# grahamstockton87/RayTracingOneWeekendApplication

Hardware: AMD Instinct MI355X
Metric: Msamples/sec (pixels x spp) on RTIOW final scene 1920x1080 (higher is better)
Workload: dtype f64; 1 GPU; book1_final 1920x1080x100spp depth 50 (BASELINE configs[1]); tiles=8x8 px per wave, interleaved over ranks, parallelism=1 GPU, scene_seed=1592598565, render_seed=1, program_ops=1337, reduced=False, variant=0, order=fast (rtk_scene_upload_fast; proven bit-identical), frames_in_flight=1

## Files before the change

include/rtk.h:

```cpp
#ifndef RTK_H
#define RTK_H

#include <stddef.h>
#include <stdint.h>

#ifdef __cplusplus
extern "C" {
#endif

#define RTK_ABI_VERSION 2

typedef enum rtk_status {
    RTK_OK = 0,
    RTK_ERR_INVALID = -1,
    RTK_ERR_NO_DEVICE = -2,
    RTK_ERR_HIP = -3,
    RTK_ERR_UNSUPPORTED = -4,
    RTK_ERR_NO_SCENE = -5
} rtk_status;

typedef struct rtk_vec3 { double x, y, z; } rtk_vec3;

typedef enum rtk_node_kind {
    RTK_NODE_SPHERE = 1,
// ... 487 lines not shown
int rtk_gather_irradiance_host(rtk_ctx* ctx, const rtk_gather_opts* opts, int64_t n, const double* h_points, const double* h_normals, double* h_irradiance);
int rtk_gather_occlusion_host(rtk_ctx* ctx, const rtk_gather_opts* opts, int64_t n, const double* h_points, const double* h_normals, double* h_open,
                              double* h_bent);

int rtk_debug_closest_hit(rtk_ctx* ctx, int real_mode, int n, const double* h_rays, const uint32_t* h_keys,
                          double* h_out, uint64_t* h_draws);

int rtk_debug_scatter(rtk_ctx* ctx, int real_mode, int n, const int32_t* h_materials, const double* h_rays, const double* h_records,
                      const uint32_t* h_keys, double* h_out, uint64_t* h_draws);
int rtk_debug_texture(rtk_ctx* ctx, int real_mode, int n, const int32_t* h_textures, const double* h_uvp, double* h_out, uint64_t* h_work);
int rtk_debug_get_ray(rtk_ctx* ctx, int real_mode, const rtk_camera* cam, uint32_t seed, int n, const int32_t* h_pixel_sample,
                      double* h_out, uint64_t* h_draws);

int rtk_scene_info(rtk_ctx* ctx, int32_t* n_program_ops, int64_t* bytes_f64, int64_t* bytes_f32);

int rtk_frame_launches(const rtk_camera* cam, const rtk_render_opts* opts);

const char* rtk_kernel_name(rtk_ctx* ctx, int real_mode, int variant);

int rtk_render_views(rtk_ctx* ctx, int32_t n_views, const rtk_camera* h_cams, const uint32_t* h_seeds ,
                     const rtk_render_opts* opts, void* d_linear, uint8_t* d_rgb8, rtk_work_counters* d_counters);
int rtk_render_views_host(rtk_ctx* ctx, int32_t n_views, const rtk_camera* h_cams, const uint32_t* h_seeds, const rtk_render_opts* opts,
                          double* h_linear, uint8_t* h_rgb8, rtk_work_counters* counters);
const char* rtk_view_kernel_name(rtk_ctx* ctx, int real_mode, int variant);

#ifdef __cplusplus
}
#endif
#endif
```

raytracingoneweekendapplication_amd/csrc/rtk_api.cpp:

```cpp
#include <hip/hip_runtime.h>

#include <algorithm>
#include <cmath>
#include <cstdarg>
#include <cstdio>
#include <cstdlib>
#include <cstring>
#include <map>
#include <new>
#include <string>
#include <vector>

#include "rtk.h"
#include "rtk_ctx.h"
#include "rtk_device_layout.h"
#include "rtk_internal.h"
#include "rtk_lds_plan.h"

namespace rtk {

thread_local std::string g_error;

int fail(int code, const char* fmt, ...) {
    char buf[512];
// ... 285 lines not shown
            cont[1] = 1.0 / s.radius;
            if (kind == OP_SPHERE_MOVING) {
                cont[2] = s.center_dir.x;
                cont[3] = s.center_dir.y;
                cont[4] = s.center_dir.z;
                cont[5] = s.radius * s.radius;
            } else {
                cont[2] = s.radius * s.radius;
            }
            rec->aux = (op.aux & 255u) | (uint32_t(s.material) << 8);
        }
    }
    extent_out = float(extent);
}

static double scene_extent(const rtk_scene_desc& sc, double eye_extent) {
    double e = eye_extent;
    auto take = [&](double v) { e = std::max(e, std::fabs(v)); };
    for (int32_t i = 0; i < sc.n_bvh_boxes; i++) {
        const rtk_aabb& b = sc.bvh_boxes[i];
        for (double v : {b.xmin, b.xmax, b.ymin, b.ymax, b.zmin, b.zmax}) take(v);
    }
    for (int32_t i = 0; i < sc.n_spheres; i++) {
        const rtk_sphere& s = sc.spheres[i];
        for (double c : {s.center0.x, s.center0.y, s.center0.z, s.center0.x + s.center_dir.x, s.center0.y + s.center_dir.y, s.center0.z + s.center_dir.z})
            e = std::max(e, std::fabs(c) + std::fabs(s.radius));
    }
    for (int32_t i = 0; i < sc.n_quads; i++) {
        const rtk_quad& q = sc.quads[i];
        for (int k = 0; k < 4; k++) {
// ... 359 lines not shown
    if ((rc = out.upload(slots, &out.view.program)) != RTK_OK) return rc;
    if ((rc = out.upload(tris, &out.view.tris)) != RTK_OK) return rc;
    if ((rc = out.upload(mats, &out.view.materials)) != RTK_OK) return rc;
    if ((rc = out.upload(texs, &out.view.textures)) != RTK_OK) return rc;
    if ((rc = out.upload(images, &out.view.images)) != RTK_OK) return rc;
    if ((rc = out.upload(texels, &out.view.texels)) != RTK_OK) return rc;
    if ((rc = out.upload(perlins, &out.view.perlins)) != RTK_OK) return rc;
    if ((rc = out.upload(chains, &out.view.chains)) != RTK_OK) return rc;
    if ((rc = out.upload(lights, &out.view.lights)) != RTK_OK) return rc;
    out.view.n_slots = int32_t(slots.size());
    out.view.n_lights = sc.n_lights;
    out.view.n_materials = sc.n_materials;
    out.view.n_perlins = sc.n_perlins;
    out.view.n_chains = int32_t(chains.size());
    out.view.program_mixed = nullptr;
    out.view.n_units = 0;
    out.view.extent = 0.0f;
    out.view.box_cache = nullptr;
    out.view.kind_words = nullptr;
    out.view.box_rank = nullptr;
    out.view.n_cached_boxes = out.view.n_kind_words = out.view.n_rank_words = 0;
    if (lds_plan::wants_box_table(slots.size() * sizeof(Slot<real>), mats.size() * sizeof(MaterialRec<real>))) {
        std::vector<BoxRec<real>> boxes;
        std::vector<uint32_t> kind_words((slots.size() + 7) / 8, 0u);
        std::vector<uint2> rank((slots.size() + 31) / 32, uint2{0u, 0u});
        for (size_t pc = 0; pc < slots.size();) {
            const uint32_t kind = slots[pc].kind_payload & 15u;
            kind_words[pc >> 3] |= kind << ((pc & 7) * 4);
            if (kind == OP_BOX) {
                rank[pc >> 5].x |= 1u << (pc & 31);
// ... 32 lines not shown
    if (fast_order) {
        std::vector<uint32_t> rank_of_slot(slots.size(), 0u);
        bool any = false;
        for (size_t i = 0; i < prog.ops.size(); i++) {
            rank_of_slot[slot_of_op[i]] = prog.ranks[i];
            any = any || prog.ranks[i] != 0;
        }
        if (any && (rc = out.upload(rank_of_slot, &out.view.tie_rank_slot)) != RTK_OK) return rc;
    }
    if constexpr (sizeof(real) == 8) {
        if (fast_order && want_mixed) {
            std::vector<MixedHead> units;
            std::vector<uint32_t> ranks;
            build_mixed_program(sc, prog, eye_extent, units, ranks, out.view.extent);
            if ((rc = out.upload(units, &out.view.program_mixed)) != RTK_OK) return rc;
            if ((rc = out.upload(ranks, &out.view.tie_rank)) != RTK_OK) return rc;
            out.view.n_units = int32_t(units.size());
        } else if (fast_order) {
            std::vector<Unit16> units;
            std::vector<uint32_t> ranks;
            build_compact_program(sc, prog, eye_extent, units, ranks, out.view.extent);
            if ((rc = out.upload(units, &out.view.program_compact)) != RTK_OK) return rc;
            if ((rc = out.upload(ranks, &out.view.tie_rank)) != RTK_OK) return rc;
            out.view.n_units16 = int32_t(units.size());
            out.view.compact_ch = compact_ch_family(prog) ? 1 : 0;
            if ((prog.features & ~kFeatQuadBox) != 0 && (prog.features & ~kFeatMesh) != 0) {
                std::vector<Unit16> hot, cold;
                std::vector<uint32_t> ranks_by_id;
                build_hot_cold_program(sc, prog, hot, cold, ranks_by_id);
                if (getenv("RTK_DEBUG")) fprintf(stderr, "[rtk] COMPACT program %zu B; hot part %zu B, cold part %zu B\n", units.size() * 16, hot.size() * 16, cold.size() * 16);
// ... 228 lines not shown
    RTK_HIP(hipSetDevice(ctx->device));
    ctx->has_scene = false;
    ctx->order_valid = false;
    const bool want_mixed = fast_order && prog.features == kFeatLean && prog.chains.size() <= 1;
    if ((rc = build_device_scene<double>(*scene, prog, ctx->scene64, fast_order, want_mixed, eye_extent)) != RTK_OK) return rc;
    if ((rc = build_device_scene<float>(*scene, prog, ctx->scene32, fast_order)) != RTK_OK) return rc;
    ctx->features = prog.features | hierarchy_flags;
    ctx->n_ops = int32_t(prog.ops.size());
    ctx->n_materials = scene->n_materials;
    ctx->n_textures = scene->n_textures;
    ctx->scene_digest = scene_digest(*scene, prog, ctx->features, fast_order, eye_extent);
    ctx->has_scene = true;
    return RTK_OK;
}

int rtk_scene_info(rtk_ctx* ctx, int32_t* n_program_ops, int64_t* bytes_f64, int64_t* bytes_f32) {
    if (!ctx || !ctx->has_scene) return fail(RTK_ERR_NO_SCENE, "rtk_scene_info: no scene uploaded");
    if (n_program_ops) *n_program_ops = ctx->scene64.view.n_slots;
    if (bytes_f64) *bytes_f64 = ctx->scene64.bytes;
    if (bytes_f32) *bytes_f32 = ctx->scene32.bytes;
    return RTK_OK;
}

}

namespace rtk {

size_t hot_program_lds_bytes(const rtk_scene_desc* scene) {
    if (!scene) return 0;
    try {
// ... 43 lines not shown
```

raytracingoneweekendapplication_amd/csrc/rtk_device_layout.h:

```cpp
#ifndef RTK_DEVICE_LAYOUT_H
#define RTK_DEVICE_LAYOUT_H

#include <stdint.h>
#include <hip/hip_vector_types.h>


namespace rtk {

enum OpKind : uint32_t {
    OP_END = 0,
    OP_BOX = 1,
    OP_SPHERE = 2,
    OP_QUAD = 3,
    OP_TRI = 4,
    OP_CHAIN = 5,
    OP_MED_BEGIN = 6,
    OP_MED_MID = 7,
    OP_MED_END = 8,
    OP_SPHERE_MOVING = 9,
    OP_MED_SPHERE = 10,
    OP_DEAD = 15
};

struct Op {
// ... 21 lines not shown
inline constexpr int slots_of(uint32_t kind) {
    return kind == OP_QUAD ? 3 : ((kind == OP_TRI || kind == OP_SPHERE_MOVING) ? 2 : 1);
}

struct alignas(16) MixedHead {
    uint32_t w[6];
    uint32_t kind_payload, aux;
    constexpr float f(int k) const { return __builtin_bit_cast(float, w[k]); }
    constexpr double d(int k) const { return __builtin_bit_cast(double, (unsigned long long)(w[2 * k]) | ((unsigned long long)(w[2 * k + 1]) << 32)); }
    void set_f(int k, float x) { w[k] = __builtin_bit_cast(uint32_t, x); }
    void set_d(int k, double x) {
        const unsigned long long v = __builtin_bit_cast(unsigned long long, x);
        w[2 * k] = uint32_t(v);
        w[2 * k + 1] = uint32_t(v >> 32);
    }
};
static_assert(sizeof(MixedHead) == 32, "mixed unit size");
inline constexpr int mixed_units(uint32_t kind) { return kind == OP_SPHERE ? 2 : (kind == OP_SPHERE_MOVING ? 3 : 1); }

struct alignas(16) Unit16 {
    uint32_t w[4];
};
inline constexpr int compact_units(uint32_t kind) {
    return (kind == OP_SPHERE || kind == OP_MED_SPHERE) ? 3 : (kind == OP_SPHERE_MOVING ? 5 : (kind == OP_QUAD ? 9 : (kind == OP_TRI ? 5 : 2)));
}

constexpr uint32_t kNoHit = 0xFFFFFFFFu;
constexpr int kMaxChain = 4;
constexpr int kMaxChunks = 64;
constexpr int kLdsBytesPerCU = 160 * 1024;

enum Feature : uint32_t {
// ... 74 lines not shown
template <typename real>
struct SceneView {
    const Slot<real>* program;
    const TriRec<real>* tris;
    const MaterialRec<real>* materials;
    const TextureRec<real>* textures;
    const ImageRec* images;
    const uint8_t* texels;
    const PerlinRec<real>* perlins;
    const ChainRec<real>* chains;
    const LightRec<real>* lights;
    int32_t n_slots, n_lights, n_materials;
    const MixedHead* program_mixed;
    int32_t n_units;
    float extent;
    const Unit16* program_compact;
    int32_t n_units16;
    int32_t compact_ch;
    const Unit16* program_hot;
    const Unit16* program_cold;
    int32_t n_hot_units, n_cold_units;
    const uint32_t* tie_rank_hot;
    const uint32_t* tie_rank;
    const uint32_t* tie_rank_slot;
    const BoxRec<real>* box_cache;
    const uint32_t* kind_words;
    const uint2* box_rank;
    int32_t n_cached_boxes, n_kind_words, n_rank_words;
    int32_t n_perlins, n_chains;
};
// ... 22 lines not shown
```

raytracingoneweekendapplication_amd/csrc/rtk_microbench.hip:

```cpp
#include <hip/hip_runtime.h>

#include <algorithm>
#include <cstdint>
#include <cstdio>
#include <cstring>
#include <vector>

namespace {

__global__ __launch_bounds__(256) void copy_kernel(const uint4* __restrict__ src, uint4* __restrict__ dst, size_t n) {
    for (size_t i = size_t(blockIdx.x) * 256 + threadIdx.x; i < n; i += size_t(gridDim.x) * 256) dst[i] = src[i];
}
__global__ __launch_bounds__(256) void read_kernel(const uint4* __restrict__ src, size_t n, unsigned* __restrict__ sink) {
    unsigned acc = 0;
    for (size_t i = size_t(blockIdx.x) * 256 + threadIdx.x; i < n; i += size_t(gridDim.x) * 256) {
        const uint4 v = src[i];
        acc ^= v.x ^ v.y ^ v.z ^ v.w;
    }
    if (acc == 0x12345u) *sink = acc;
}

template <bool RANDOM>
__global__ __launch_bounds__(1024) void lds_read_kernel(int iters, unsigned* __restrict__ sink) {
    extern __shared__ __align__(16) unsigned char lds[];
// ... 24 lines not shown
                                                       unsigned long long* __restrict__ real_ticks = nullptr) {
    __shared__ unsigned next[4096];
    for (int k = threadIdx.x; k < 4096; k += 64) next[k] = (k * 1031u + 17u) & 4095u;
    __syncthreads();
    unsigned at = threadIdx.x;
    const unsigned long long r0 = __builtin_amdgcn_s_memrealtime();
    const unsigned long long t0 = __builtin_amdgcn_s_memtime();
    for (int it = 0; it < iters; it++) at = next[at];
    const unsigned long long t1 = __builtin_amdgcn_s_memtime();
    const unsigned long long r1 = __builtin_amdgcn_s_memrealtime();
    if (threadIdx.x == 0) cycles[blockIdx.x] = t1 - t0;
    if (threadIdx.x == 0 && real_ticks) real_ticks[blockIdx.x] = r1 - r0;
    if (at == 0xFFFFFFFFu) *sink = at;
}

enum IssueClass { I_FMA_F32, I_FMA_F64, I_MUL_F64, I_ADD_F64, I_MUL_LO_U32, I_RCP_F32, I_SQRT_F32, I_RCP_F64, I_RSQ_F64, I_SQRT_F64, I_CNDMASK, I_MAX3_F32, I_PK_FMA_F32, I_PK_MUL_F32, I_FMAC_F32, I_MUL_F32, I_COUNT };

constexpr int kIssueReps = 16;
template <int CLS>
__global__ __launch_bounds__(1024) void issue_kernel(int iters, unsigned long long* __restrict__ cycles, float* __restrict__ sink,
                                                    unsigned long long* __restrict__ real_ticks = nullptr) {
    float f[8];
    double d[8];
    unsigned u[8];
    for (int k = 0; k < 8; k++) {
        f[k] = 1.0f + 0.001f * float(threadIdx.x + k);
        d[k] = 1.0 + 0.001 * double(threadIdx.x + k);
        u[k] = threadIdx.x * 3u + unsigned(k) + 1u;
    }
    const float fb = 0.999f, fc = 0.001f;
    const double db = 0.999, dc = 0.001;
    const unsigned um = 0x9E3779B1u;
    const unsigned long long r0 = __builtin_amdgcn_s_memrealtime();
    const unsigned long long t0 = __builtin_amdgcn_s_memtime();
    for (int it = 0; it < iters; it++) {
#pragma unroll
        for (int rep = 0; rep < kIssueReps; rep++) {
#pragma unroll
            for (int k = 0; k < 8; k++) {
                if (CLS == I_FMA_F32) asm volatile("v_fma_f32 %0, %0, %1, %2" : "+v"(f[k]) : "v"(fb), "v"(fc));
                if (CLS == I_FMA_F64) asm volatile("v_fma_f64 %0, %0, %1, %2" : "+v"(d[k]) : "v"(db), "v"(dc));
                if (CLS == I_MUL_F64) asm volatile("v_mul_f64 %0, %0, %1" : "+v"(d[k]) : "v"(db));
                if (CLS == I_ADD_F64) asm volatile("v_add_f64 %0, %0, %1" : "+v"(d[k]) : "v"(dc));
                if (CLS == I_MUL_LO_U32) asm volatile("v_mul_lo_u32 %0, %0, %1" : "+v"(u[k]) : "v"(um));
                if (CLS == I_RCP_F32) asm volatile("v_rcp_f32 %0, %0" : "+v"(f[k]));
                if (CLS == I_SQRT_F32) asm volatile("v_sqrt_f32 %0, %0" : "+v"(f[k]));
                if (CLS == I_RCP_F64) asm volatile("v_rcp_f64 %0, %0" : "+v"(d[k]));
                if (CLS == I_RSQ_F64) asm volatile("v_rsq_f64 %0, %0" : "+v"(d[k]));
                if (CLS == I_SQRT_F64) asm volatile("v_sqrt_f64 %0, %0" : "+v"(d[k]));
                if (CLS == I_CNDMASK) asm volatile("v_cndmask_b32 %0, %0, %1, vcc" : "+v"(f[k]) : "v"(fb));
                if (CLS == I_MAX3_F32) asm volatile("v_max3_f32 %0, %0, %1, %2" : "+v"(f[k]) : "v"(fb), "v"(fc));
                if (CLS == I_PK_FMA_F32) asm volatile("v_pk_fma_f32 %0, %0, %1, %2" : "+v"(d[k]) : "v"(db), "v"(dc));
                if (CLS == I_PK_MUL_F32) asm volatile("v_pk_mul_f32 %0, %0, %1" : "+v"(d[k]) : "v"(db));
                if (CLS == I_FMAC_F32) asm volatile("v_fmac_f32 %0, %1, %2" : "+v"(f[k]) : "v"(fb), "v"(fc));
                if (CLS == I_MUL_F32) asm volatile("v_mul_f32 %0, %0, %1" : "+v"(f[k]) : "v"(fb));
            }
        }
    }
    const unsigned long long t1 = __builtin_amdgcn_s_memtime();
    const unsigned long long r1 = __builtin_amdgcn_s_memrealtime();
    if (threadIdx.x == 0) cycles[blockIdx.x] = t1 - t0;
    if (threadIdx.x == 0 && real_ticks) real_ticks[blockIdx.x] = r1 - r0;
    float acc = 0.0f;
    for (int k = 0; k < 8; k++) acc += f[k] + float(d[k]) + float(u[k]);
    if (acc == 12345.678f) *sink = acc;
}

const char* kNames =
    "hbm_copy_GBps,hbm_read_GBps,lds_read_b128_GBps,lds_read_b128_random_GBps,lds_roundtrip_cycles,shader_clock_GHz,"
    "issue_v_fma_f32,issue_v_fma_f64,issue_v_mul_f64,issue_v_add_f64,issue_v_mul_lo_u32,issue_v_rcp_f32,issue_v_sqrt_f32,issue_v_rcp_f64,issue_v_rsq_f64,"
    "issue_v_sqrt_f64,issue_v_cndmask_b32,issue_v_max3_f32,issue_v_pk_fma_f32,issue_v_pk_mul_f32,issue_v_fmac_f32,issue_v_mul_f32,clock_dense_valu_GHz,clock_light_load_GHz,"
    "issue_v_fma_f32_1wave,issue_v_fma_f32_2waves,issue_v_fma_f32_4waves,issue_v_fma_f32_8waves";
constexpr int kResults = 6 + I_COUNT + 2 + 4;

#define MB_HIP(call)                                  \
    do {                                              \
        const hipError_t e_ = (call);                 \
        if (e_ != hipSuccess) {                       \
            std::snprintf(g_err, sizeof g_err, "%s: %s", #call, hipGetErrorString(e_)); \
            return -3;                                \
        }                                             \
    } while (0)
char g_err[256] = "";

template <typename F>
int time_ms(F&& launch, int reps, float* best_ms) {
// ... 116 lines not shown
    if (rc == 0) rc = run_issue<I_FMA_F64>(cus, bw, bt, d_cycles, d_real, d_fsink, &out[6 + I_FMA_F64], nullptr);
    if (rc == 0) rc = run_issue<I_MUL_F64>(cus, bw, bt, d_cycles, d_real, d_fsink, &out[6 + I_MUL_F64], nullptr);
    if (rc == 0) rc = run_issue<I_ADD_F64>(cus, bw, bt, d_cycles, d_real, d_fsink, &out[6 + I_ADD_F64], nullptr);
    if (rc == 0) rc = run_issue<I_MUL_LO_U32>(cus, bw, bt, d_cycles, d_real, d_fsink, &out[6 + I_MUL_LO_U32], nullptr);
    if (rc == 0) rc = run_issue<I_RCP_F32>(cus, bw, bt, d_cycles, d_real, d_fsink, &out[6 + I_RCP_F32], nullptr);
    if (rc == 0) rc = run_issue<I_SQRT_F32>(cus, bw, bt, d_cycles, d_real, d_fsink, &out[6 + I_SQRT_F32], nullptr);
    if (rc == 0) rc = run_issue<I_RCP_F64>(cus, bw, bt, d_cycles, d_real, d_fsink, &out[6 + I_RCP_F64], nullptr);
    if (rc == 0) rc = run_issue<I_RSQ_F64>(cus, bw, bt, d_cycles, d_real, d_fsink, &out[6 + I_RSQ_F64], nullptr);
    if (rc == 0) rc = run_issue<I_SQRT_F64>(cus, bw, bt, d_cycles, d_real, d_fsink, &out[6 + I_SQRT_F64], nullptr);
    if (rc == 0) rc = run_issue<I_CNDMASK>(cus, bw, bt, d_cycles, d_real, d_fsink, &out[6 + I_CNDMASK], nullptr);
    if (rc == 0) rc = run_issue<I_MAX3_F32>(cus, bw, bt, d_cycles, d_real, d_fsink, &out[6 + I_MAX3_F32], nullptr);
    if (rc == 0) rc = run_issue<I_PK_FMA_F32>(cus, bw, bt, d_cycles, d_real, d_fsink, &out[6 + I_PK_FMA_F32], nullptr);
    if (rc == 0) rc = run_issue<I_PK_MUL_F32>(cus, bw, bt, d_cycles, d_real, d_fsink, &out[6 + I_PK_MUL_F32], nullptr);
    if (rc == 0) rc = run_issue<I_FMAC_F32>(cus, bw, bt, d_cycles, d_real, d_fsink, &out[6 + I_FMAC_F32], nullptr);
    if (rc == 0) rc = run_issue<I_MUL_F32>(cus, bw, bt, d_cycles, d_real, d_fsink, &out[6 + I_MUL_F32], nullptr);
    if (rc == 0) {
        const int blocks = cus * bw, iters = 40000 / kIssueReps;
        for (int k = 0; k < 100; k++) issue_kernel<I_FMA_F32><<<dim3(blocks), dim3(bt), 0, nullptr>>>(iters, d_cycles, d_fsink, d_real);
        MB_HIP(hipDeviceSynchronize());
        rc = clock_from(d_cycles, d_real, blocks, &out[6 + I_COUNT]);
        if (rc == 0) {
            lds_chain_kernel<<<dim3(cus), dim3(64), 0, nullptr>>>(200000, d_cycles, sink, d_real);
            MB_HIP(hipDeviceSynchronize());
            rc = clock_from(d_cycles, d_real, cus, &out[6 + I_COUNT + 1]);
        }
    }
    (void)hipFree(d_real);
    (void)hipFree(src);
    (void)hipFree(dst);
    (void)hipFree(sink);
// ... 7 lines not shown
```

raytracingoneweekendapplication_amd/csrc/rtk_render_body.inc:

```
    extern __shared__ __align__(16) unsigned char lds_program[];
    if constexpr (IN_LDS) {
        typedef const unsigned char __attribute__((address_space(3))) * lds_bytes_t;
        if (uint32_t(size_t((lds_bytes_t)lds_program)) != 0u) return;
    }
    constexpr bool BRACKET = (FEAT_ALL & F_SPHERE_MEDIA_ONLY) == 0;
    constexpr uint32_t FEAT = FEAT_ALL & ~uint32_t(F_LDS_BOXES | F_SPHERE_MEDIA_ONLY) & ~uint32_t(RTK_DEV_MASK_OFF);
    constexpr bool LDS_PART = (FEAT_ALL & F_LDS_BOXES) != 0;
    static_assert(!LDS_PART || !IN_LDS, "F_LDS_BOXES: for programs that do not fit LDS");
    constexpr bool MIXED = (FEAT & F_F32_BOX) != 0;
    constexpr bool COMPACT = MIXED && (FEAT & ~uint32_t(F_F32_BOX | F_MATTE)) != kFeatLean;
    static_assert(!MIXED || sizeof(real) == 8, "F_F32_BOX: f64 kernels only");
    constexpr bool CH = MIXED && !COMPACT;
    constexpr bool CHE = COMPACT && kCompactChStatic<FEAT>;
    constexpr bool CHE_RT = COMPACT && COUNT && !CHE;
    [[maybe_unused]] const bool che_rt = CHE_RT && sc.compact_ch != 0;
    constexpr int kCulling = CH ? 1 : (CHE ? 2 : (CHE_RT ? 3 : 0));
    constexpr bool SPLIT = LDS_PART && !COMPACT;
    constexpr bool COLD = LDS_PART && COMPACT;
    static_assert(!LDS_PART || !MIXED || COMPACT, "F_LDS_BOXES with f32 boxes: the COMPACT program");
    constexpr bool XF = (FEAT & F_XFORM) != 0;
    using ProgRec = std::conditional_t<COMPACT, Unit16, std::conditional_t<MIXED, MixedHead, Slot<real>>>;
    using CurRec = std::conditional_t<MIXED, MixedHead, Slot<real>>;
    constexpr uint32_t kBoxUnits = COMPACT ? 2u : 1u, kSphereUnits = COMPACT ? 3u : (MIXED ? 2u : 1u), kQuadUnits = COMPACT ? 9u : 3u, kTriUnits = COMPACT ? 5u : 2u;
    const ProgRec* prog;
    if constexpr (COLD) prog = sc.program_hot;
    else if constexpr (COMPACT) prog = sc.program_compact;
    else if constexpr (MIXED) prog = sc.program_mixed;
    else prog = sc.program;
    const int n_records = COLD ? sc.n_hot_units : (COMPACT ? sc.n_units16 : (MIXED ? sc.n_units : sc.n_slots));
    [[maybe_unused]] const Unit16* cold = nullptr;
    if constexpr (COLD) cold = sc.program_cold;
    const MaterialRec<real>* mats = sc.materials;
    if constexpr (IN_LDS || COLD) {
        const int n_prog16 = n_records * int(sizeof(ProgRec) / 16);
        const int n_mat16 = sc.n_materials * int(sizeof(MaterialRec<real>) / 16);
        const uint4* __restrict__ src = reinterpret_cast<const uint4*>(prog);
        const uint4* __restrict__ msrc = reinterpret_cast<const uint4*>(sc.materials);
        uint4* dst = reinterpret_cast<uint4*>(lds_program);
        for (int k = threadIdx.x; k < n_prog16; k += blockDim.x) dst[k] = src[k];
        for (int k = threadIdx.x; k < n_mat16; k += blockDim.x) dst[n_prog16 + k] = msrc[k];
        if constexpr (COLD && (FEAT & F_TEXTURE) != 0) {
// ... 51 lines not shown
    constexpr uint32_t kPcUnit = CH ? kChPcUnit : 1u;
    auto rec_at = [&](uint32_t pc) -> const ProgRec* {
        if constexpr (CH && IN_LDS) {
            typedef const unsigned char __attribute__((address_space(3))) * lds_bytes_t;
            return reinterpret_cast<const ProgRec*>((const unsigned char*)(lds_bytes_t)(size_t)pc);
        } else if constexpr (CH) return reinterpret_cast<const ProgRec*>(reinterpret_cast<const unsigned char*>(prog) + pc);
        else return prog + pc;
    };
    auto head_at = [&](uint32_t pc) -> CurRec {
        if constexpr (COMPACT) return *reinterpret_cast<const MixedHead*>(prog + (pc & kPcMask));
        else return *rec_at(pc);
    };
    auto kind_of = [&](uint32_t pc) -> uint32_t {
        if constexpr (SPLIT) return (lds_kinds[pc >> 3] >> ((pc & 7u) * 4u)) & 15u;
        else if constexpr (COMPACT) return prog[(pc & kPcMask) + 1].w[2] & 15u;
        else return rec_at(pc)->kind_payload & 15u;
    };
    [[maybe_unused]] auto box_at = [&](uint32_t pc) -> CurRec {
        const uint2 e = lds_rank[pc >> 5];
        const uint32_t at = e.y + uint32_t(__builtin_popcount(e.x & ((1u << (pc & 31u)) - 1u)));
        if constexpr (MIXED) {
            return CurRec{};
        } else {
            const BoxRec<real> b = lds_boxes[at];
            Slot<real> s;
            #pragma unroll
            for (int k = 0; k < 6; k++) s.v[k] = b.v[k];
            s.kind_payload = OP_BOX;
            s.aux = b.aux;
            return s;
// ... 174 lines not shown
        if ((m_box | m_sph | m_oth | m_shd | m_quad | m_tri) == 0ull) {
            if (exhausted) break;
            continue;
        }
        const int n_box = popcount64(m_box), n_sph = popcount64(m_sph), n_oth = popcount64(m_oth), n_shd = popcount64(m_shd);
        const int n_quad = popcount64(m_quad), n_tri = popcount64(m_tri);
        RTK_PROF_MARK(0, 1, n_box + n_sph + n_oth + n_shd + n_quad + n_tri)
        int pick;
        if (n_box >= n_sph && n_box >= n_quad && n_box >= n_tri && n_box >= n_shd && n_box >= n_oth) pick = W_BOX;
        else if (n_sph >= n_quad && n_sph >= n_tri && n_sph >= n_shd && n_sph >= n_oth) pick = W_SPHERE;
        else if (n_quad >= n_tri && n_quad >= n_shd && n_quad >= n_oth) pick = W_QUAD;
        else if (n_tri >= n_shd && n_tri >= n_oth) pick = W_TRI;
        else if (n_shd >= n_oth) pick = W_SHADE;
        else pick = W_OTHER;
        if (pick == W_BOX) {
            const int sel = int(diag >> 8) & 7;
            const int eighths = sel == 0 ? (kFamily == kFeatMesh ? 3 : 2) : sel;
            const int frac = (n_box * eighths) >> 3;
            const int keep = frac > 8 ? frac : 8;
            constexpr int kBoxUnroll = COLD ? kUnrollCold : SPLIT ? kUnrollSplit
                                       : (((MIXED && !COMPACT) || FEAT == (kFeatLean | uint32_t(F_FMA_BOX))) ? kUnrollMixed
                                          : (kFamily == kFeatAll ? 2 : (kFamily == kFeatQuadBox ? (COMPACT ? kUnrollCompactQuadBox : kUnrollQuadBox)
                                                                       : (kFamily == kFeatMesh ? (COMPACT ? kUnrollCompactMesh : kUnrollMesh) : kUnrollLean))));
            CurRec cur;
            uint32_t k = kind;
            auto fetch = [&]() {
                if constexpr (SPLIT) {
                    k = kind_of(L.pc);
                    if (k == OP_BOX) cur = box_at(L.pc);
                } else {
// ... 69 lines not shown
                    }
                }
                if constexpr ((FEAT & ~uint32_t(F_FMA_BOX | F_F32_BOX | F_MATTE)) == kFeatQuadBox) {
                    if (popcount64(__ballot(k == OP_QUAD)) >= kQuadRide) {
                        if (k == OP_QUAD) {
                            hit_quad<XF, MIXED>(L, prog + L.pc, kQuadUnits, cnt, tie);
                            fetch();
                            L.kind = k;
                        }
                    }
                }
                remaining = popcount64(__ballot(k == box_kind));
                RTK_PROF_MARK(1, 1, remaining)
            } while (remaining >= keep);
            __builtin_amdgcn_s_setprio(0);
        } else if (pick == W_SPHERE) {
            const int ssel = int(diag >> 11) & 7;
            const int sfrac = (n_sph * (ssel == 0 ? 4 : ssel)) >> 3;
            const int keep = sfrac > 8 ? sfrac : 8;
            CurRec cur = head_at(L.pc);
            uint32_t k = kind;
            int remaining;
            __builtin_amdgcn_s_setprio(kSphereLoopPrio);
            do {
                if (k == OP_SPHERE) {
                    if constexpr (COMPACT) step_sphere_compact<XF>(L, cur, prog + L.pc, cnt, tie);
                    else if constexpr (MIXED) step_sphere_mixed<kPcUnit>(L, cur, rec_at(L.pc), cnt, tie, extent);
                    else step_sphere<XF>(L, cur, cnt, tie);
                    if constexpr (SPLIT) {
                        k = kind_of(L.pc);
                        if (k == OP_SPHERE) cur = head_at(L.pc);
                    } else {
                        cur = head_at(L.pc);
                        k = cur.kind_payload & 15u;
                    }
                    L.kind = k;
                }
                remaining = popcount64(__ballot(k == OP_SPHERE));
                RTK_PROF_MARK(2, 1, remaining)
            } while (remaining >= keep);
            __builtin_amdgcn_s_setprio(0);
        } else if ((FEAT & F_QUAD) && pick == W_QUAD) {
          if constexpr ((FEAT & F_QUAD) != 0) {
            const int keep = (n_quad >> 1) > 8 ? (n_quad >> 1) : 8;
            uint32_t k = kind;
            int remaining;
            __builtin_amdgcn_s_setprio(kPrimLoopPrio);
            do {
                if (k == OP_QUAD) {
// ... 115 lines not shown
```

raytracingoneweekendapplication_amd/csrc/rtk_trace.hip:

```cpp
#include <hip/hip_runtime.h>

#include <cstdio>
#include <cstdlib>
#include <type_traits>

#include "rtk.h"
#include "rtk_device_layout.h"
#include "rtk_device_math.h"
#include "rtk_gather_rule.h"
#include "rtk_image_pass.h"
#include "rtk_lds_plan.h"
#include "rtk_trace.h"

namespace rtk {

template <typename real> RTK_DEV V3<real> ld3(const real* p) { return V3<real>{p[0], p[1], p[2]}; }
template <typename real> RTK_DEV V3<real> operator-(V3<real> a) { return V3<real>{-a.x, -a.y, -a.z}; }
template <typename real> RTK_DEV V3<real> operator-(V3<real> a, V3<real> b) { return V3<real>{a.x - b.x, a.y - b.y, a.z - b.z}; }
template <typename real> RTK_DEV V3<real> operator*(V3<real> a, V3<real> b) { return V3<real>{a.x * b.x, a.y * b.y, a.z * b.z}; }
template <typename real> RTK_DEV V3<real> divide(V3<real> a, real t) { return scale(real(1) / t, a); }
template <typename real> RTK_DEV real dot(V3<real> a, V3<real> b) { return a.x * b.x + a.y * b.y + a.z * b.z; }
template <typename real> RTK_DEV V3<real> cross(V3<real> a, V3<real> b) {
    return V3<real>{a.y * b.z - a.z * b.y, a.z * b.x - a.x * b.z, a.x * b.y - a.y * b.x};
}
// ... 510 lines not shown
RTK_DEV float min3_clamp01(float a, float b, float c) { float r; asm("v_min3_f32 %0, %1, %2, %3 clamp" : "=v"(r) : "v"(a), "v"(b), "v"(c)); return r; }
RTK_DEV bool slab_test32_chs(const MixedHead& b, V3<float> oi, V3<float> inv) {
    const float tcx = __builtin_fmaf(b.f(0), inv.x, -oi.x), tcy = __builtin_fmaf(b.f(1), inv.y, -oi.y), tcz = __builtin_fmaf(b.f(2), inv.z, -oi.z);
    const float ax = __builtin_fabsf(inv.x), ay = __builtin_fabsf(inv.y), az = __builtin_fabsf(inv.z);
    const float nx = __builtin_fmaf(-b.f(3), ax, tcx), fx = __builtin_fmaf(b.f(3), ax, tcx);
    const float ny = __builtin_fmaf(-b.f(4), ay, tcy), fy = __builtin_fmaf(b.f(4), ay, tcy);
    const float nz = __builtin_fmaf(-b.f(5), az, tcz), fz = __builtin_fmaf(b.f(5), az, tcz);
    return min3_clamp01(fx, fy, fz) > max3_clamp01(nx, ny, nz);
}
template <typename real, bool COUNT>
RTK_DEV void step_box32_ch(Lane<real>& L, const MixedHead& rec, Counters<COUNT>& cnt) {
    cnt.inc(C_BOX);
    const bool hit = slab_test32_chs(rec, L.oi32s, L.inv32s);
    L.pc = hit ? L.pc + kChPcUnit : rec.aux;
}
template <bool XF = false, uint32_t UNITS = 1, uint32_t PCU = 1, typename real, bool COUNT>
RTK_DEV void step_box_mixed_exact(Lane<real>& L, const MixedHead& rec, Counters<COUNT>& cnt, bool compact_ch = false) {
    cnt.inc(C_BOX);
    Slot<real> b;
    if (UNITS == 1 || (UNITS == 2 && compact_ch)) {
        for (int k = 0; k < 3; k++) {
            b.v[2 * k] = real(rec.f(k)) - real(rec.f(3 + k));
            b.v[2 * k + 1] = real(rec.f(k)) + real(rec.f(3 + k));
        }
    } else {
        for (int k = 0; k < 6; k++) b.v[k] = real(rec.f(k));
    }
    const V3<real> d = ray_d<XF>(L);
    const V3<real> inv = mk(real(1) / d.x, real(1) / d.y, real(1) / d.z);
    const bool hit = slab_test<true>(b, ray_o<XF>(L), inv, L.tmin, L.best_t);
    L.pc = hit ? L.pc + UNITS * PCU : rec.aux;
}
template <uint32_t PCU = 1, typename real, bool COUNT, typename Tie>
RTK_DEV void step_sphere_mixed(Lane<real>& L, const MixedHead& head, const MixedHead* __restrict__ rec, Counters<COUNT>& cnt, const Tie& tie, float extent) {
    const double radius2 = reinterpret_cast<const double*>(rec + 1)[2];
    hit_sphere<false, true, true, true>(L, mk(real(head.d(0)), real(head.d(1)), real(head.d(2))), real(radius2), 2u * PCU, cnt, tie, extent);
}
template <bool XF, typename real, bool COUNT, typename Tie>
RTK_DEV void step_sphere_compact(Lane<real>& L, const MixedHead& head, const Unit16* __restrict__ rec, Counters<COUNT>& cnt, const Tie& tie) {
    hit_sphere<XF, true>(L, mk(real(head.d(0)), real(head.d(1)), real(head.d(2))), packed<real, 3>(rec) * packed<real, 3>(rec), 3u, cnt, tie);
}
template <uint32_t PCU = 1, typename real, bool COUNT, typename Tie>
RTK_DEV void step_other_mixed(Lane<real>& L, const MixedHead* __restrict__ rec, Counters<COUNT>& cnt, const Tie& tie, float extent) {
    const uint32_t kind = rec->kind_payload & 15u;
    if (kind == OP_BOX) {
        step_box_mixed_exact<false, 1, PCU>(L, *rec, cnt);
    } else if (kind == OP_SPHERE_MOVING) {
        const double* cont = reinterpret_cast<const double*>(rec + 1);
        const V3<real> cc = mk(real(rec->d(0)), real(rec->d(1)), real(rec->d(2))) + scale(L.tm, mk(real(cont[2]), real(cont[3]), real(cont[4])));
        hit_sphere<false, true, true, true>(L, cc, real(cont[5]), 3u * PCU, cnt, tie, extent);
    } else {
        L.pc += uint32_t(mixed_units(kind)) * PCU;
    }
}
template <bool EXACT_NAN, bool XF, bool FMA = false, typename real, bool COUNT>
RTK_DEV void step_box(Lane<real>& L, const Slot<real>& rec, Counters<COUNT>& cnt) {
    cnt.inc(C_BOX);
    bool hit;
    if constexpr (FMA && !EXACT_NAN) hit = slab_test_fma(rec, L.oi, L.inv, L.tmin, L.best_t);
    else hit = slab_test<EXACT_NAN>(rec, ray_o<XF>(L), L.inv, L.tmin, L.best_t);
    L.pc = hit ? L.pc + 1 : rec.aux;
// ... 222 lines not shown
#else
#define RTK_SHADE_PROF_PARAM
#define RTK_SHADE_PROF_ARG
#define RTK_SHADE_PROF_BEGIN
#define RTK_SHADE_PROF(k)
#endif

template <typename real>
struct Surface {
    V3<real> p, normal;
    real u, v;
    int material;
    bool front_face;
};

template <typename real>
RTK_DEV void make_surface_mixed(const MixedHead* __restrict__ prog, uint32_t best_pc, real t, V3<real> wo, V3<real> wd, real tm, Surface<real>& sf) {
    const MixedHead* rec = prog + best_pc;
    const uint32_t kind = rec->kind_payload & 15u;
    const double* cont = reinterpret_cast<const double*>(rec + 1);
    sf.material = int(rec->aux >> 8);
    sf.p = wo + scale(t, wd);
    sf.u = real(0);
    sf.v = real(0);
    V3<real> cc = mk(real(rec->d(0)), real(rec->d(1)), real(rec->d(2)));
    if (kind == OP_SPHERE_MOVING) cc = cc + scale(tm, mk(real(cont[2]), real(cont[3]), real(cont[4])));
    const V3<real> outward = scale(real(cont[1]), sf.p - cc);
    sf.front_face = dot(wd, outward) < real(0);
    sf.normal = sf.front_face ? outward : -outward;
}


template <typename real, typename Rec>
RTK_DEV void tri_barycentrics(const Rec* __restrict__ rec, real ox, real oy, real oz, real dx, real dy, real dz, float* fa, float* fb, float* fg) {
    real tt;
    float a = 0, b = 0, g = 0;
// ... 191 lines not shown
    return L.depth <= 0;
}

template <typename real, uint32_t FEAT, bool COUNT, typename ProgT>
RTK_DEV bool shade(Lane<real>& L, const ProgT* __restrict__ hit_rec, const SceneView<real>& sc, const MaterialRec<real>* __restrict__ mats,
                   const CameraRec<real>& cam, Counters<COUNT>& cnt RTK_SHADE_PROF_PARAM) {
    RTK_SHADE_PROF_BEGIN
    if (L.best_pc == kNoHit) {
        if constexpr (kNoRadianceState<FEAT>) L.sum = L.sum + L.throughput * ld3(cam.background);
        else L.radiance = L.radiance + L.throughput * ld3(cam.background);
        return true;
    }
    cnt.inc(C_SURFACE);
    RTK_SHADE_PROF(2)
    Surface<real> sf;
    if constexpr (std::is_same_v<ProgT, MixedHead>) make_surface_mixed(hit_rec, 0u, L.best_t, L.ro, L.rd, L.tm, sf);
    else make_surface<real, FEAT>(hit_rec, sc, mats, 0u, L.best_t, L.ro, L.rd, L.tm, sf);
    RTK_SHADE_PROF(0)
    return shade_surface<real, FEAT>(L, sf, sc, mats, cnt RTK_SHADE_PROF_ARG);
}

enum Want : int { W_DONE = 0, W_BOX = 1, W_SPHERE = 2, W_OTHER = 3, W_SHADE = 4, W_QUAD = 5, W_TRI = 6 };

RTK_DEV bool uniform(bool c) { return __builtin_amdgcn_readfirstlane(int(c)) != 0; }

RTK_DEV int popcount64(unsigned long long m) {
    int n;
    asm("s_bcnt1_i32_b64 %0, %1" : "=s"(n) : "s"(m) : "scc");
    return n;
}

// ... 1287 lines not shown
template hipError_t launch_lens_guides<double>(const SceneView<double>&, const LensRec&, const CameraRec<double>&, uint32_t, int, int, int, float*, hipStream_t);
template hipError_t launch_lens_guides<float>(const SceneView<float>&, const LensRec&, const CameraRec<float>&, uint32_t, int, int, int, float*, hipStream_t);

#ifdef RTK_ISA_PROBES
constexpr uint32_t kProbeFeat = kFeatLean | uint32_t(F_F32_BOX);
enum ProbeKind : int { PROBE_EMPTY, PROBE_BOX, PROBE_SPHERE, PROBE_SEGMENT, PROBE_SAMPLE, PROBE_MISS, PROBE_LAMBERTIAN, PROBE_METAL, PROBE_DIELECTRIC, PROBE_PARTIAL };
template <int KIND>
__global__ __launch_bounds__(1024) void rtk_isa_probe(Lane<double>* __restrict__ lanes, const MixedHead* __restrict__ prog, SceneView<double> sc,
                                                       const CameraRec<double>* __restrict__ cam_ptr, double* __restrict__ partial, float extent) {
    const int gid = blockIdx.x * 1024 + threadIdx.x;
    Lane<double> L = lanes[gid];
    Counters<false> cnt;
    const NoTie tie{};
    const MixedHead* rec = reinterpret_cast<const MixedHead*>(reinterpret_cast<const unsigned char*>(prog) + L.pc);
    if constexpr (KIND == PROBE_BOX) {
        MixedHead cur = *rec;
        step_box32_ch(L, cur, cnt);
        cur = *reinterpret_cast<const MixedHead*>(reinterpret_cast<const unsigned char*>(prog) + L.pc);
        L.kind = cur.kind_payload & 15u;
        L.oi32_lo.x = cur.f(0);
    } else if constexpr (KIND == PROBE_SPHERE) {
        MixedHead cur = *rec;
        step_sphere_mixed<kChPcUnit>(L, cur, rec, cnt, tie, extent);
        cur = *reinterpret_cast<const MixedHead*>(reinterpret_cast<const unsigned char*>(prog) + L.pc);
        L.kind = cur.kind_payload & 15u;
        L.oi32_lo.x = cur.f(0);
    } else if constexpr (KIND == PROBE_SEGMENT) {
        begin_segment<false, true, 1>(L, cnt, extent);
        L.kind = rec->kind_payload & 15u;
    } else if constexpr (KIND == PROBE_SAMPLE) {
        begin_sample(L, *cam_ptr, int(L.segs), L.depth, pcg_hash(L.best_pc), cnt);
    } else if constexpr (KIND == PROBE_MISS) {
        L.sum = L.sum + L.throughput * ld3(cam_ptr->background);
    } else if constexpr (KIND == PROBE_LAMBERTIAN || KIND == PROBE_METAL || KIND == PROBE_DIELECTRIC) {
        Surface<double> sf;
// ... 26 lines not shown
```

Baseline: 11800 Msamples/s.

## Repack mixed program into LDS image layout with kind in first quad

Builds a second copy of the mixed sphere/box program whose 32-byte units are reordered so the box link and kind sit in the first 16-byte word, and uses it when the program lives in LDS. The box traversal loop fetches two b128 LDS loads directly and decodes kind from the first quad, avoiding extra dependent loads and repacking per step. Sphere, shading and other paths are templated to read either layout. It adds a second program upload, an XOR-encoded kind field, and a debug export API, plus an fma_mix microbench entry.

```diff
diff --git a/include/rtk.h b/include/rtk.h
--- a/include/rtk.h
+++ b/include/rtk.h
@@ -525,6 +525,9 @@
 
 int rtk_scene_info(rtk_ctx* ctx, int32_t* n_program_ops, int64_t* bytes_f64, int64_t* bytes_f32);
 
+int rtk_debug_mixed_program(const rtk_scene_desc* optimized, double eye_extent, int32_t capacity_units, int32_t* n_units, float* extent, void* h_units,
+                            void* h_image);
+
 int rtk_frame_launches(const rtk_camera* cam, const rtk_render_opts* opts);
 
 const char* rtk_kernel_name(rtk_ctx* ctx, int real_mode, int variant);
diff --git a/raytracingoneweekendapplication_amd/csrc/rtk_api.cpp b/raytracingoneweekendapplication_amd/csrc/rtk_api.cpp
--- a/raytracingoneweekendapplication_amd/csrc/rtk_api.cpp
+++ b/raytracingoneweekendapplication_amd/csrc/rtk_api.cpp
@@ -323,6 +323,27 @@
     extent_out = float(extent);
 }
 
+static void build_mixed_lds_image(const std::vector<MixedHead>& units, std::vector<MixedImg>& image) {
+    image.assign(units.size(), MixedImg{});
+    std::memcpy(image.data(), units.data(), units.size() * sizeof(MixedHead));
+    for (size_t u = 0; u < units.size();) {
+        const MixedHead& src = units[u];
+        MixedImg& dst = image[u];
+        const uint32_t kind = src.kind_payload & 15u;
+        if (kind == OP_BOX) {
+            for (int k = 0; k < 3; k++) dst.w[k] = src.w[k], dst.w[4 + k] = src.w[3 + k];
+            dst.w[3] = src.aux;
+            dst.w[7] = src.kind_payload;
+        } else {
+            dst.w[0] = src.w[0], dst.w[1] = src.w[1];
+            dst.w[2] = src.aux;
+            dst.w[3] = src.kind_payload ^ kImageKindXor;
+            for (int k = 0; k < 4; k++) dst.w[4 + k] = src.w[2 + k];
+        }
+        u += size_t(mixed_units(kind));
+    }
+}
+
 static double scene_extent(const rtk_scene_desc& sc, double eye_extent) {
     double e = eye_extent;
     auto take = [&](double v) { e = std::max(e, std::fabs(v)); };
@@ -712,6 +733,7 @@
     out.view.n_perlins = sc.n_perlins;
     out.view.n_chains = int32_t(chains.size());
     out.view.program_mixed = nullptr;
+    out.view.program_mixed_lds = nullptr;
     out.view.n_units = 0;
     out.view.extent = 0.0f;
     out.view.box_cache = nullptr;
@@ -774,6 +796,9 @@
             std::vector<uint32_t> ranks;
             build_mixed_program(sc, prog, eye_extent, units, ranks, out.view.extent);
             if ((rc = out.upload(units, &out.view.program_mixed)) != RTK_OK) return rc;
+            std::vector<MixedImg> image;
+            build_mixed_lds_image(units, image);
+            if ((rc = out.upload(image, &out.view.program_mixed_lds)) != RTK_OK) return rc;
             if ((rc = out.upload(ranks, &out.view.tie_rank)) != RTK_OK) return rc;
             out.view.n_units = int32_t(units.size());
         } else if (fast_order) {
@@ -1032,6 +1057,34 @@
     return RTK_OK;
 }
 
+int rtk_debug_mixed_program(const rtk_scene_desc* optimized, double eye_extent, int32_t capacity_units, int32_t* n_units, float* extent, void* h_units,
+                            void* h_image) {
+    if (!optimized || !n_units) return fail(RTK_ERR_INVALID, "rtk_debug_mixed_program: null argument");
+    try {
+        Program prog;
+        const int rc = compile_scene(optimized, prog);
+        if (rc != RTK_OK) return rc;
+        if (prog.features != kFeatLean || prog.chains.size() > 1) return fail(RTK_ERR_INVALID, "rtk_debug_mixed_program: not a sphere-only scene");
+        std::vector<MixedHead> units;
+        std::vector<uint32_t> ranks;
+        float ext = 0.0f;
+        build_mixed_program(*optimized, prog, eye_extent, units, ranks, ext);
+        *n_units = int32_t(units.size());
+        if (extent) *extent = ext;
+        if (size_t(capacity_units < 0 ? 0 : capacity_units) < units.size() && (h_units || h_image))
+            return fail(RTK_ERR_INVALID, "rtk_debug_mixed_program: %zu units, room for %d", units.size(), capacity_units);
+        if (h_units) std::memcpy(h_units, units.data(), units.size() * sizeof(MixedHead));
+        if (h_image) {
+            std::vector<MixedImg> image;
+            build_mixed_lds_image(units, image);
+            std::memcpy(h_image, image.data(), image.size() * sizeof(MixedImg));
+        }
+        return RTK_OK;
+    } catch (const std::bad_alloc&) {
+        return fail(RTK_ERR_INVALID, "rtk_debug_mixed_program: out of memory");
+    }
+}
+
 int rtk_scene_info(rtk_ctx* ctx, int32_t* n_program_ops, int64_t* bytes_f64, int64_t* bytes_f32) {
     if (!ctx || !ctx->has_scene) return fail(RTK_ERR_NO_SCENE, "rtk_scene_info: no scene uploaded");
     if (n_program_ops) *n_program_ops = ctx->scene64.view.n_slots;
diff --git a/raytracingoneweekendapplication_amd/csrc/rtk_device_layout.h b/raytracingoneweekendapplication_amd/csrc/rtk_device_layout.h
--- a/raytracingoneweekendapplication_amd/csrc/rtk_device_layout.h
+++ b/raytracingoneweekendapplication_amd/csrc/rtk_device_layout.h
@@ -59,8 +59,23 @@
         w[2 * k] = uint32_t(v);
         w[2 * k + 1] = uint32_t(v >> 32);
     }
+    constexpr uint32_t kind() const { return kind_payload & 15u; }
+    constexpr uint32_t aux_word() const { return aux; }
 };
 static_assert(sizeof(MixedHead) == 32, "mixed unit size");
+constexpr uint32_t kImageKindXor = 1u;
+struct alignas(16) MixedImg {
+    uint32_t w[8];
+    constexpr double d(int k) const {
+        const int at = k == 0 ? 0 : 2 + 2 * k;
+        return __builtin_bit_cast(double, (unsigned long long)(w[at]) | ((unsigned long long)(w[at + 1]) << 32));
+    }
+    constexpr float f(int k) const { return __builtin_bit_cast(float, w[k < 3 ? k : k + 1]); }
+    constexpr uint32_t kind() const { return (w[3] & 15u) ^ kImageKindXor; }
+    constexpr uint32_t aux_word() const { return w[2]; }
+    constexpr uint32_t link() const { return w[3]; }
+};
+static_assert(sizeof(MixedImg) == 32, "mixed unit size");
 inline constexpr int mixed_units(uint32_t kind) { return kind == OP_SPHERE ? 2 : (kind == OP_SPHERE_MOVING ? 3 : 1); }
 
 struct alignas(16) Unit16 {
@@ -165,6 +180,7 @@
     const MixedHead* program_mixed;
     int32_t n_units;
     float extent;
+    const MixedImg* program_mixed_lds;
     const Unit16* program_compact;
     int32_t n_units16;
     int32_t compact_ch;
diff --git a/raytracingoneweekendapplication_amd/csrc/rtk_microbench.hip b/raytracingoneweekendapplication_amd/csrc/rtk_microbench.hip
--- a/raytracingoneweekendapplication_amd/csrc/rtk_microbench.hip
+++ b/raytracingoneweekendapplication_amd/csrc/rtk_microbench.hip
@@ -62,7 +62,7 @@
     if (at == 0xFFFFFFFFu) *sink = at;
 }
 
-enum IssueClass { I_FMA_F32, I_FMA_F64, I_MUL_F64, I_ADD_F64, I_MUL_LO_U32, I_RCP_F32, I_SQRT_F32, I_RCP_F64, I_RSQ_F64, I_SQRT_F64, I_CNDMASK, I_MAX3_F32, I_PK_FMA_F32, I_PK_MUL_F32, I_FMAC_F32, I_MUL_F32, I_COUNT };
+enum IssueClass { I_FMA_F32, I_FMA_F64, I_MUL_F64, I_ADD_F64, I_MUL_LO_U32, I_RCP_F32, I_SQRT_F32, I_RCP_F64, I_RSQ_F64, I_SQRT_F64, I_CNDMASK, I_MAX3_F32, I_PK_FMA_F32, I_PK_MUL_F32, I_FMAC_F32, I_MUL_F32, I_FMA_MIX_F32, I_COUNT };
 
 constexpr int kIssueReps = 16;
 template <int CLS>
@@ -79,6 +79,7 @@
     const float fb = 0.999f, fc = 0.001f;
     const double db = 0.999, dc = 0.001;
     const unsigned um = 0x9E3779B1u;
+    const unsigned hb = 0x3BFE3BFEu;
     const unsigned long long r0 = __builtin_amdgcn_s_memrealtime();
     const unsigned long long t0 = __builtin_amdgcn_s_memtime();
     for (int it = 0; it < iters; it++) {
@@ -102,6 +103,7 @@
                 if (CLS == I_PK_MUL_F32) asm volatile("v_pk_mul_f32 %0, %0, %1" : "+v"(d[k]) : "v"(db));
                 if (CLS == I_FMAC_F32) asm volatile("v_fmac_f32 %0, %1, %2" : "+v"(f[k]) : "v"(fb), "v"(fc));
                 if (CLS == I_MUL_F32) asm volatile("v_mul_f32 %0, %0, %1" : "+v"(f[k]) : "v"(fb));
+                if (CLS == I_FMA_MIX_F32) asm volatile("v_fma_mix_f32 %0, %1, %0, %2 op_sel_hi:[1,0,0]" : "+v"(f[k]) : "v"(hb), "v"(fc));
             }
         }
     }
@@ -117,7 +119,7 @@
 const char* kNames =
     "hbm_copy_GBps,hbm_read_GBps,lds_read_b128_GBps,lds_read_b128_random_GBps,lds_roundtrip_cycles,shader_clock_GHz,"
     "issue_v_fma_f32,issue_v_fma_f64,issue_v_mul_f64,issue_v_add_f64,issue_v_mul_lo_u32,issue_v_rcp_f32,issue_v_sqrt_f32,issue_v_rcp_f64,issue_v_rsq_f64,"
-    "issue_v_sqrt_f64,issue_v_cndmask_b32,issue_v_max3_f32,issue_v_pk_fma_f32,issue_v_pk_mul_f32,issue_v_fmac_f32,issue_v_mul_f32,clock_dense_valu_GHz,clock_light_load_GHz,"
+    "issue_v_sqrt_f64,issue_v_cndmask_b32,issue_v_max3_f32,issue_v_pk_fma_f32,issue_v_pk_mul_f32,issue_v_fmac_f32,issue_v_mul_f32,issue_v_fma_mix_f32,clock_dense_valu_GHz,clock_light_load_GHz,"
     "issue_v_fma_f32_1wave,issue_v_fma_f32_2waves,issue_v_fma_f32_4waves,issue_v_fma_f32_8waves";
 constexpr int kResults = 6 + I_COUNT + 2 + 4;
 
@@ -264,6 +266,7 @@
     if (rc == 0) rc = run_issue<I_PK_MUL_F32>(cus, bw, bt, d_cycles, d_real, d_fsink, &out[6 + I_PK_MUL_F32], nullptr);
     if (rc == 0) rc = run_issue<I_FMAC_F32>(cus, bw, bt, d_cycles, d_real, d_fsink, &out[6 + I_FMAC_F32], nullptr);
     if (rc == 0) rc = run_issue<I_MUL_F32>(cus, bw, bt, d_cycles, d_real, d_fsink, &out[6 + I_MUL_F32], nullptr);
+    if (rc == 0) rc = run_issue<I_FMA_MIX_F32>(cus, bw, bt, d_cycles, d_real, d_fsink, &out[6 + I_FMA_MIX_F32], nullptr);
     if (rc == 0) {
         const int blocks = cus * bw, iters = 40000 / kIssueReps;
         for (int k = 0; k < 100; k++) issue_kernel<I_FMA_F32><<<dim3(blocks), dim3(bt), 0, nullptr>>>(iters, d_cycles, d_fsink, d_real);
diff --git a/raytracingoneweekendapplication_amd/csrc/rtk_render_body.inc b/raytracingoneweekendapplication_amd/csrc/rtk_render_body.inc
--- a/raytracingoneweekendapplication_amd/csrc/rtk_render_body.inc
+++ b/raytracingoneweekendapplication_amd/csrc/rtk_render_body.inc
@@ -11,6 +11,7 @@
     constexpr bool COMPACT = MIXED && (FEAT & ~uint32_t(F_F32_BOX | F_MATTE)) != kFeatLean;
     static_assert(!MIXED || sizeof(real) == 8, "F_F32_BOX: f64 kernels only");
     constexpr bool CH = MIXED && !COMPACT;
+    constexpr bool IMG = CH && IN_LDS;
     constexpr bool CHE = COMPACT && kCompactChStatic<FEAT>;
     constexpr bool CHE_RT = COMPACT && COUNT && !CHE;
     [[maybe_unused]] const bool che_rt = CHE_RT && sc.compact_ch != 0;
@@ -19,12 +20,13 @@
     constexpr bool COLD = LDS_PART && COMPACT;
     static_assert(!LDS_PART || !MIXED || COMPACT, "F_LDS_BOXES with f32 boxes: the COMPACT program");
     constexpr bool XF = (FEAT & F_XFORM) != 0;
-    using ProgRec = std::conditional_t<COMPACT, Unit16, std::conditional_t<MIXED, MixedHead, Slot<real>>>;
-    using CurRec = std::conditional_t<MIXED, MixedHead, Slot<real>>;
+    using ProgRec = std::conditional_t<COMPACT, Unit16, std::conditional_t<MIXED, std::conditional_t<IMG, MixedImg, MixedHead>, Slot<real>>>;
+    using CurRec = std::conditional_t<MIXED, std::conditional_t<IMG, MixedImg, MixedHead>, Slot<real>>;
     constexpr uint32_t kBoxUnits = COMPACT ? 2u : 1u, kSphereUnits = COMPACT ? 3u : (MIXED ? 2u : 1u), kQuadUnits = COMPACT ? 9u : 3u, kTriUnits = COMPACT ? 5u : 2u;
     const ProgRec* prog;
     if constexpr (COLD) prog = sc.program_hot;
     else if constexpr (COMPACT) prog = sc.program_compact;
+    else if constexpr (IMG) prog = sc.program_mixed_lds;
     else if constexpr (MIXED) prog = sc.program_mixed;
     else prog = sc.program;
     const int n_records = COLD ? sc.n_hot_units : (COMPACT ? sc.n_units16 : (MIXED ? sc.n_units : sc.n_slots));
@@ -106,6 +108,7 @@
     auto kind_of = [&](uint32_t pc) -> uint32_t {
         if constexpr (SPLIT) return (lds_kinds[pc >> 3] >> ((pc & 7u) * 4u)) & 15u;
         else if constexpr (COMPACT) return prog[(pc & kPcMask) + 1].w[2] & 15u;
+        else if constexpr (MIXED) return rec_at(pc)->kind();
         else return rec_at(pc)->kind_payload & 15u;
     };
     [[maybe_unused]] auto box_at = [&](uint32_t pc) -> CurRec {
@@ -310,6 +313,45 @@
         else if (n_shd >= n_oth) pick = W_SHADE;
         else pick = W_OTHER;
         if (pick == W_BOX) {
+          if constexpr (IMG) {
+            const int sel = int(diag >> 8) & 7;
+            const int frac = (n_box * (sel == 0 ? 2 : sel)) >> 3;
+            const int keep = frac > 8 ? frac : 8;
+            typedef const rtk_u32x4 __attribute__((address_space(3))) * lds_uint4_t;
+            rtk_u32x4 a, b;
+            uint32_t k = kind ^ kImageKindXor;
+            auto fetch = [&]() {
+                a = *(lds_uint4_t)(size_t)L.pc;
+                b = *(lds_uint4_t)(size_t)(L.pc + 16u);
+                k = a.w & 15u;
+            };
+            a = *(lds_uint4_t)(size_t)L.pc;
+            b = *(lds_uint4_t)(size_t)(L.pc + 16u);
+            const uint32_t box_code = L.box_kind ^ kImageKindXor;
+            constexpr uint32_t sphere_code = uint32_t(OP_SPHERE) ^ kImageKindXor;
+            int remaining;
+            __builtin_amdgcn_s_setprio(kBoxLoopPrio);
+            do {
+                #pragma unroll
+                for (int step = 0; step < kUnrollMixed; step++) {
+                    if (k == box_code) {
+                        step_box_img(L, a, b, cnt);
+                        fetch();
+                    }
+                }
+                if ([[maybe_unused]] const int n_ride = popcount64(__ballot(k == sphere_code)); n_ride >= sphere_min) {
+                    if (k == sphere_code) {
+                        step_sphere_img<kPcUnit>(L, a, b, rec_at(L.pc), cnt, tie, extent);
+                        fetch();
+                    }
+                    RTK_PROF_MARK(2, 1, n_ride)
+                }
+                remaining = popcount64(__ballot(k == box_code));
+                RTK_PROF_MARK(1, 1, remaining)
+            } while (remaining >= keep);
+            __builtin_amdgcn_s_setprio(0);
+            L.kind = k ^ kImageKindXor;
+          } else {
             const int sel = int(diag >> 8) & 7;
             const int eighths = sel == 0 ? (kFamily == kFeatMesh ? 3 : 2) : sel;
             const int frac = (n_box * eighths) >> 3;
@@ -409,6 +451,7 @@
                 RTK_PROF_MARK(1, 1, remaining)
             } while (remaining >= keep);
             __builtin_amdgcn_s_setprio(0);
+          }
         } else if (pick == W_SPHERE) {
             const int ssel = int(diag >> 11) & 7;
             const int sfrac = (n_sph * (ssel == 0 ? 4 : ssel)) >> 3;
@@ -427,7 +470,8 @@
                         if (k == OP_SPHERE) cur = head_at(L.pc);
                     } else {
                         cur = head_at(L.pc);
-                        k = cur.kind_payload & 15u;
+                        if constexpr (IMG) k = cur.kind();
+                        else k = cur.kind_payload & 15u;
                     }
                     L.kind = k;
                 }
diff --git a/raytracingoneweekendapplication_amd/csrc/rtk_trace.hip b/raytracingoneweekendapplication_amd/csrc/rtk_trace.hip
--- a/raytracingoneweekendapplication_amd/csrc/rtk_trace.hip
+++ b/raytracingoneweekendapplication_amd/csrc/rtk_trace.hip
@@ -548,6 +548,16 @@
     const bool hit = slab_test32_chs(rec, L.oi32s, L.inv32s);
     L.pc = hit ? L.pc + kChPcUnit : rec.aux;
 }
+typedef uint32_t rtk_u32x4 __attribute__((ext_vector_type(4)));
+template <typename real, bool COUNT>
+RTK_DEV void step_box_img(Lane<real>& L, rtk_u32x4 a, rtk_u32x4 b, Counters<COUNT>& cnt) {
+    cnt.inc(C_BOX);
+    const uint32_t a0 = a.x, a1 = a.y, a2 = a.z, b0 = b.x, b1 = b.y, b2 = b.z;
+    MixedHead rec;
+    rec.w[0] = a0, rec.w[1] = a1, rec.w[2] = a2, rec.w[3] = b0, rec.w[4] = b1, rec.w[5] = b2;
+    const bool hit = slab_test32_chs(rec, L.oi32s, L.inv32s);
+    L.pc = hit ? L.pc + kChPcUnit : a.w;
+}
 template <bool XF = false, uint32_t UNITS = 1, uint32_t PCU = 1, typename real, bool COUNT>
 RTK_DEV void step_box_mixed_exact(Lane<real>& L, const MixedHead& rec, Counters<COUNT>& cnt, bool compact_ch = false) {
     cnt.inc(C_BOX);
@@ -565,20 +575,36 @@
     const bool hit = slab_test<true>(b, ray_o<XF>(L), inv, L.tmin, L.best_t);
     L.pc = hit ? L.pc + UNITS * PCU : rec.aux;
 }
-template <uint32_t PCU = 1, typename real, bool COUNT, typename Tie>
-RTK_DEV void step_sphere_mixed(Lane<real>& L, const MixedHead& head, const MixedHead* __restrict__ rec, Counters<COUNT>& cnt, const Tie& tie, float extent) {
+template <uint32_t PCU = 1, typename real, bool COUNT, typename Tie, typename Rec>
+RTK_DEV void step_sphere_mixed(Lane<real>& L, const Rec& head, const Rec* __restrict__ rec, Counters<COUNT>& cnt, const Tie& tie, float extent) {
     const double radius2 = reinterpret_cast<const double*>(rec + 1)[2];
     hit_sphere<false, true, true, true>(L, mk(real(head.d(0)), real(head.d(1)), real(head.d(2))), real(radius2), 2u * PCU, cnt, tie, extent);
+}
+template <uint32_t PCU = 1, typename real, bool COUNT, typename Tie>
+RTK_DEV void step_sphere_img(Lane<real>& L, rtk_u32x4 a, rtk_u32x4 b, const MixedImg* __restrict__ rec, Counters<COUNT>& cnt, const Tie& tie, float extent) {
+    const double radius2 = reinterpret_cast<const double*>(rec + 1)[2];
+    const unsigned long long xw = (unsigned long long)(a.x) | ((unsigned long long)(a.y) << 32);
+    const unsigned long long yw = (unsigned long long)(b.x) | ((unsigned long long)(b.y) << 32);
+    const unsigned long long zw = (unsigned long long)(b.z) | ((unsigned long long)(b.w) << 32);
+    const double cx = __builtin_bit_cast(double, xw), cy = __builtin_bit_cast(double, yw), cz = __builtin_bit_cast(double, zw);
+    hit_sphere<false, true, true, true>(L, mk(real(cx), real(cy), real(cz)), real(radius2), 2u * PCU, cnt, tie, extent);
 }
 template <bool XF, typename real, bool COUNT, typename Tie>
 RTK_DEV void step_sphere_compact(Lane<real>& L, const MixedHead& head, const Unit16* __restrict__ rec, Counters<COUNT>& cnt, const Tie& tie) {
     hit_sphere<XF, true>(L, mk(real(head.d(0)), real(head.d(1)), real(head.d(2))), packed<real, 3>(rec) * packed<real, 3>(rec), 3u, cnt, tie);
 }
-template <uint32_t PCU = 1, typename real, bool COUNT, typename Tie>
-RTK_DEV void step_other_mixed(Lane<real>& L, const MixedHead* __restrict__ rec, Counters<COUNT>& cnt, const Tie& tie, float extent) {
-    const uint32_t kind = rec->kind_payload & 15u;
+template <uint32_t PCU = 1, typename real, bool COUNT, typename Tie, typename Rec>
+RTK_DEV void step_other_mixed(Lane<real>& L, const Rec* __restrict__ rec, Counters<COUNT>& cnt, const Tie& tie, float extent) {
+    const uint32_t kind = rec->kind();
     if (kind == OP_BOX) {
-        step_box_mixed_exact<false, 1, PCU>(L, *rec, cnt);
+        if constexpr (std::is_same_v<Rec, MixedImg>) {
+            MixedHead box;
+            for (int k = 0; k < 6; k++) box.w[k] = __builtin_bit_cast(uint32_t, rec->f(k));
+            box.aux = rec->link();
+            step_box_mixed_exact<false, 1, PCU>(L, box, cnt);
+        } else {
+            step_box_mixed_exact<false, 1, PCU>(L, *rec, cnt);
+        }
     } else if (kind == OP_SPHERE_MOVING) {
         const double* cont = reinterpret_cast<const double*>(rec + 1);
         const V3<real> cc = mk(real(rec->d(0)), real(rec->d(1)), real(rec->d(2))) + scale(L.tm, mk(real(cont[2]), real(cont[3]), real(cont[4])));
@@ -831,12 +857,12 @@
     bool front_face;
 };
 
-template <typename real>
-RTK_DEV void make_surface_mixed(const MixedHead* __restrict__ prog, uint32_t best_pc, real t, V3<real> wo, V3<real> wd, real tm, Surface<real>& sf) {
-    const MixedHead* rec = prog + best_pc;
-    const uint32_t kind = rec->kind_payload & 15u;
+template <typename real, typename Rec>
+RTK_DEV void make_surface_mixed(const Rec* __restrict__ prog, uint32_t best_pc, real t, V3<real> wo, V3<real> wd, real tm, Surface<real>& sf) {
+    const Rec* rec = prog + best_pc;
+    const uint32_t kind = rec->kind();
     const double* cont = reinterpret_cast<const double*>(rec + 1);
-    sf.material = int(rec->aux >> 8);
+    sf.material = int(rec->aux_word() >> 8);
     sf.p = wo + scale(t, wd);
     sf.u = real(0);
     sf.v = real(0);
@@ -1058,7 +1084,7 @@
     cnt.inc(C_SURFACE);
     RTK_SHADE_PROF(2)
     Surface<real> sf;
-    if constexpr (std::is_same_v<ProgT, MixedHead>) make_surface_mixed(hit_rec, 0u, L.best_t, L.ro, L.rd, L.tm, sf);
+    if constexpr (std::is_same_v<ProgT, MixedHead> || std::is_same_v<ProgT, MixedImg>) make_surface_mixed(hit_rec, 0u, L.best_t, L.ro, L.rd, L.tm, sf);
     else make_surface<real, FEAT>(hit_rec, sc, mats, 0u, L.best_t, L.ro, L.rd, L.tm, sf);
     RTK_SHADE_PROF(0)
     return shade_surface<real, FEAT>(L, sf, sc, mats, cnt RTK_SHADE_PROF_ARG);
@@ -2376,11 +2402,13 @@
     const NoTie tie{};
     const MixedHead* rec = reinterpret_cast<const MixedHead*>(reinterpret_cast<const unsigned char*>(prog) + L.pc);
     if constexpr (KIND == PROBE_BOX) {
-        MixedHead cur = *rec;
-        step_box32_ch(L, cur, cnt);
-        cur = *reinterpret_cast<const MixedHead*>(reinterpret_cast<const unsigned char*>(prog) + L.pc);
-        L.kind = cur.kind_payload & 15u;
-        L.oi32_lo.x = cur.f(0);
+        const rtk_u32x4* at = reinterpret_cast<const rtk_u32x4*>(rec);
+        rtk_u32x4 a = at[0], b = at[1];
+        step_box_img(L, a, b, cnt);
+        at = reinterpret_cast<const rtk_u32x4*>(reinterpret_cast<const unsigned char*>(prog) + L.pc);
+        a = at[0], b = at[1];
+        L.kind = a.w & 15u;
+        L.oi32_lo.x = __builtin_bit_cast(float, uint32_t(a.x)) + __builtin_bit_cast(float, uint32_t(b.x));
     } else if constexpr (KIND == PROBE_SPHERE) {
         MixedHead cur = *rec;
         step_sphere_mixed<kChPcUnit>(L, cur, rec, cnt, tie, extent);
```

Result: faster. 11960 Msamples/s (median of 6 runs) (+1.3%).
